# JohnsonLabJanelia/laserCalib

Hardware: NVIDIA B200
Metric: LM_iters_per_sec (higher is better)
Workload: dtype f64

## Files before the change

include/lcba.h:

```cpp
#ifndef LCBA_H
#define LCBA_H

#include <stddef.h>
#include <stdint.h>

#ifdef __cplusplus
extern "C" {
#endif

#define LCBA_VERSION 100
#define LCBA_CAM_PARAMS 11
#define LCBA_MAX_CAMERAS 64
#define LCBA_MAX_TRACE 512

enum {
  LCBA_OK = 0,
  LCBA_E_ARG = -1,
  LCBA_E_CUDA = -2,
  LCBA_E_STATE = -3,
  LCBA_E_UNSUPPORTED = -4,
  LCBA_E_NONFINITE = -5,
  LCBA_E_NCCL = -6
};

// ... 100 lines not shown

int lcba_nccl_unique_id(void* id_out128);
int lcba_comm_init(lcba_t* h, int32_t rank, int32_t nranks, const void* id128);

int lcba_debug_tr2d(double B00, double B01, double B11, double g0, double g1, double Delta,
                    double* p_out2, int* newton_out);

int lcba_debug_chol(lcba_t* h, int32_t n, const double* A, const double* rhs, double mu, const double* d,
                    int32_t grid, double* x_out, double* factor_out, int32_t* fail_out);

#define LCBA_STEP_SCALARS 18
int lcba_debug_step(lcba_t* h, double lam, double mu, int32_t mode, double* pc_out, double* pp_out,
                    double* scalars_out);

int lcba_debug_schur_stats(lcba_t* h, long long* out, int max_ctas, int* nkinds, int* nslices);

int lcba_debug_mma_plan(int32_t C, int32_t sm_count, int32_t* units_out, int32_t max_kinds,
                        int32_t* nslices_out, int32_t* ok_out);

int lcba_debug_i8_plan(int32_t C, int64_t P, int32_t sm_count, int32_t* tiles_out, int32_t max_tiles,
                       int32_t* work_out, int32_t max_work, int32_t* nwork_out, int32_t* nrg_out,
                       int64_t* nkb_out);

int lcba_debug_i8_fallback(lcba_t* h);

int lcba_debug_peer_reduce(lcba_t* h, int enable);

int lcba_host_is_nondecreasing_i64(const int64_t* v, int64_t n, int32_t threads);

#ifdef __cplusplus
}
#endif
#endif
```

lasercalib_b200/_cabi.py:

```python
from __future__ import annotations

import ctypes as C
import os

import numpy as np

_PKG = os.path.dirname(os.path.abspath(__file__))
LIB_PATH = os.path.join(_PKG, "liblcba.so")

LCBA_MAX_TRACE = 512
E_NAMES = {-1: "LCBA_E_ARG", -2: "LCBA_E_CUDA", -3: "LCBA_E_STATE", -4: "LCBA_E_UNSUPPORTED",
           -5: "LCBA_E_NONFINITE", -6: "LCBA_E_NCCL"}

SYMBOLS = ["lcba_version", "lcba_create", "lcba_destroy", "lcba_last_error", "lcba_default_options",
           "lcba_set_problem", "lcba_set_problem_shard", "lcba_set_params", "lcba_get_params", "lcba_rotate", "lcba_project",
           "lcba_unproject", "lcba_residuals", "lcba_jacobian_blocks", "lcba_sparsity_indices", "lcba_solve",
           "lcba_get_trace", "lcba_get_grad", "lcba_get_profile", "lcba_linearize",
           "lcba_time_device", "lcba_nccl_unique_id", "lcba_comm_init", "lcba_debug_tr2d",
           "lcba_sq_normal", "lcba_debug_schur_stats", "lcba_debug_mma_plan",
           "lcba_set_iteration_callback", "lcba_debug_i8_plan", "lcba_host_is_nondecreasing_i64", "lcba_debug_peer_reduce",
           "lcba_debug_i8_fallback", "lcba_debug_chol", "lcba_debug_step"]

STEP_SCALARS = ["reg_term", "Delta", "Jg2", "aa", "ab", "bb", "JAA", "JAB", "JBB", "gtgt", "gtp", "pp",
                "c0", "c1", "predicted", "step_h_norm", "step_norm", "chol_fail"]


class Options(C.Structure):
    _fields_ = [("ftol", C.c_double), ("xtol", C.c_double), ("gtol", C.c_double),
                ("max_nfev", C.c_int64), ("verbose", C.c_int32), ("profile", C.c_int32),
                ("max_iterations", C.c_int32), ("fix_cameras", C.c_int32), ("shared_intrinsics", C.c_int32), ("reserved", C.c_int32 * 3)]


class TraceRow(C.Structure):
    _fields_ = [("iteration", C.c_int64), ("nfev", C.c_int64), ("cost", C.c_double),
                ("cost_reduction", C.c_double), ("step_norm", C.c_double),
                ("optimality", C.c_double), ("delta", C.c_double), ("reg_term", C.c_double)]


class Result(C.Structure):
    _fields_ = [("cost", C.c_double), ("optimality", C.c_double), ("initial_cost", C.c_double),
                ("nfev", C.c_int64), ("njev", C.c_int64), ("iterations", C.c_int64),
                ("status", C.c_int32), ("n_trace", C.c_int32), ("solve_ms", C.c_double),
                ("gpu_launches", C.c_int64), ("reserved", C.c_double * 6)]

# ... 41 lines not shown
    lib.lcba_set_problem.argtypes = [vp, i32, i64, i64, vp, vp, vp, vp, vp, vp]
    lib.lcba_set_problem_shard.argtypes = [vp, i32, i64, i64, vp, vp, vp, vp, vp, vp, i64]
    lib.lcba_set_params.argtypes = [vp, vp, vp]
    lib.lcba_get_params.argtypes = [vp, vp, vp]
    lib.lcba_rotate.argtypes = [vp, i64, vp, vp, vp]
    lib.lcba_project.argtypes = [vp, i64, vp, vp, vp]
    lib.lcba_unproject.argtypes = [vp, i64, vp, vp, i64, vp, vp, vp, vp, vp]
    lib.lcba_residuals.argtypes = [vp, vp, vp, pd]
    lib.lcba_jacobian_blocks.argtypes = [vp, vp, vp, vp]
    lib.lcba_sparsity_indices.argtypes = [vp, i32, i64, i64, vp, vp, vp]
    lib.lcba_solve.argtypes = [vp, C.POINTER(Options), C.POINTER(Result)]
    lib.lcba_get_trace.argtypes = [vp, C.POINTER(TraceRow), i32]
    lib.lcba_set_iteration_callback.argtypes = [vp, ITERATION_CB, vp]
    lib.lcba_get_grad.argtypes = [vp, vp]
    lib.lcba_get_profile.argtypes = [vp, C.POINTER(KernelStat), i32, C.POINTER(i32)]
    lib.lcba_linearize.argtypes = [vp, dbl, vp, vp, vp, vp, pd]
    lib.lcba_time_device.argtypes = [vp, i32, i32, pd]
    lib.lcba_nccl_unique_id.argtypes = [vp]
    lib.lcba_comm_init.argtypes = [vp, i32, i32, vp]
    lib.lcba_sq_normal.argtypes = [vp, i32, vp, pd, vp, vp]
    lib.lcba_debug_mma_plan.argtypes = [i32, i32, vp, i32, C.POINTER(i32), C.POINTER(i32)]
    lib.lcba_debug_schur_stats.argtypes = [vp, vp, C.c_int, C.POINTER(C.c_int), C.POINTER(C.c_int)]
    lib.lcba_debug_i8_plan.argtypes = [i32, i64, i32, vp, i32, vp, i32, C.POINTER(i32), C.POINTER(i32), C.POINTER(i64)]
    lib.lcba_host_is_nondecreasing_i64.argtypes = [vp, i64, i32]
    lib.lcba_debug_peer_reduce.argtypes = [vp, i32]
    lib.lcba_debug_i8_fallback.argtypes = [vp]
    lib.lcba_debug_tr2d.argtypes = [dbl, dbl, dbl, dbl, dbl, dbl, pd, C.POINTER(C.c_int)]
    lib.lcba_debug_chol.argtypes = [vp, i32, vp, vp, dbl, vp, i32, vp, vp, C.POINTER(i32)]
    lib.lcba_debug_step.argtypes = [vp, dbl, dbl, i32, vp, vp, vp]
    _lib = lib
    return lib


def _ptr(a):
    return None if a is None else a.ctypes.data_as(C.c_void_p)


def _f64(a, shape=None):
    a = np.ascontiguousarray(a, dtype=np.float64)
    if shape is not None:
        a = a.reshape(shape)
    return a


def _i64(a):
    return np.ascontiguousarray(a, dtype=np.int64)
# ... 161 lines not shown
        return g

    def profile(self):
        stats = (KernelStat * 64)()
        n = C.c_int32()
        self._check(self.lib.lcba_get_profile(self.h, stats, 64, C.byref(n)))
        return {s.name.decode(): dict(launches=s.launches, total_ms=s.total_ms)
                for s in stats[:n.value]}

    def linearize(self, lam):
        n = 11 * self.C
        S = np.empty((n, n))
        rhs = np.empty(n)
        g = np.empty(n + 3 * self.P)
        sc = np.empty(n + 3 * self.P)
        cost = C.c_double()
        self._check(self.lib.lcba_linearize(self.h, float(lam), _ptr(S), _ptr(rhs), _ptr(g),
                                            _ptr(sc), C.byref(cost)))
        return dict(S=S, rhs=rhs, grad=g, scale_inv=sc, cost=cost.value)

    def i8_fell_back(self):
        return self.lib.lcba_debug_i8_fallback(self.h)

    def debug_chol(self, A, rhs, mu=0.0, d=None, grid=0):
        A = _f64(A)
        n = A.shape[0]
        if A.shape != (n, n):
            raise ValueError("A must be square")
        rhs = _f64(rhs).ravel()
        d = None if d is None else _f64(d).ravel()
        if rhs.size != n or (d is not None and d.size != n):
            raise ValueError("rhs and d must have n entries")
        x = np.empty(n)
        factor = np.empty((n + 1, n))
        fail = C.c_int32()
        self._check(self.lib.lcba_debug_chol(self.h, n, _ptr(A), _ptr(rhs), float(mu), _ptr(d), int(grid),
                                             _ptr(x), _ptr(factor), C.byref(fail)))
        return x, factor, fail.value

    STEP_FULL, STEP_FIX_CAMERAS, STEP_SHARED_INTRINSICS = 0, 1, 2

    def debug_step(self, lam, mu=0.0, mode=0):
        pc = np.empty(11 * self.C)
        pp = np.empty(3 * self.P)
        sc = np.empty(len(STEP_SCALARS))
        self._check(self.lib.lcba_debug_step(self.h, float(lam), float(mu), int(mode), _ptr(pc), _ptr(pp), _ptr(sc)))
# ... 28 lines not shown
```

lasercalib_b200/csrc/lcba.cu:

```cuda
#include <dlfcn.h>
#include <math.h>
#include <stdio.h>
#include <string.h>
#include <algorithm>
#include <map>
#include <string>
#include <thread>
#include <vector>

#include <nvtx3/nvToolsExt.h>

#include "common.cuh"
#include "control.cuh"
#include "dense.cuh"
#include "eval.cuh"
#include "ingest.cuh"
#include "linearize.cuh"
#include "dense_passes.cuh"
#include "schur.cuh"
#include "schur_mma.cuh"
#include "schur_i8.cuh"
#include "peer_reduce.cuh"
#include "variants.cuh"

// ... 504 lines not shown
  h->plan = make_schur_plan(C, h->sm_count, h->smem_optin - 2048);
  LCBA_TRY(dev_alloc(h, &h->d_kinds, h->plan.kinds.size()));
  LCBA_TRY(dev_alloc(h, &h->d_hws, h->plan.hws.size()));
  LCBA_CUDA(h, cudaMemcpyAsync(h->d_kinds, h->plan.kinds.data(), h->plan.kinds.size() * sizeof(SchurKind),
                               cudaMemcpyHostToDevice, st));
  LCBA_CUDA(h, cudaMemcpyAsync(h->d_hws, h->plan.hws.data(), h->plan.hws.size() * sizeof(SchurHw),
                               cudaMemcpyHostToDevice, st));
  LCBA_TRY(dev_alloc(h, &h->d_Sred, h->plan.part_stride));
  h->use_mma = false;
  h->d_mkinds = nullptr; h->d_U = nullptr; h->d_Upart = nullptr; h->d_Yg = nullptr;
  int max_slices = h->plan.nslices;
  {
    const char* de = getenv("LCBA_MMA_DENSITY");
    const double min_density = de ? atof(de) : 0.25;
    const bool dense = (double)h->n_pairs >= min_density * (double)P * C;
    const char* env = getenv("LCBA_SCHUR_MMA");
    const bool want = env ? atoi(env) != 0 : (dense && C >= 8);
    if (want && C <= MMA_MAX_CAMERAS) {
      {
        const char* ie = getenv("LCBA_SCHUR_I8");
        h->use_i8 = ie ? atoi(ie) != 0 : P >= 32768;
      }
      if (h->use_i8) {
        h->i8plan = make_i8_plan(C, P, h->sm_count);
        const I8Plan& ip = h->i8plan;
        h->i8_groups = (C + I8_GROUP_CAMS - 1) / I8_GROUP_CAMS;
        h->i8_gx_max = (int)std::max<long long>(1, std::min<long long>(ip.nkb, (long long)h->sm_count * 4 / h->i8_groups));
        h->i8_gx_make = (int)std::max<long long>(1, std::min<long long>(ip.nkb, (long long)h->sm_count * 3 / h->i8_groups));
        LCBA_TRY(dev_alloc(h, &h->d_i8work, ip.work.size()));
        LCBA_TRY(dev_alloc(h, &h->d_i8tiles, ip.tiles.size()));
        LCBA_CUDA(h, cudaMemcpyAsync(h->d_i8work, ip.work.data(), ip.work.size() * sizeof(I8Work), cudaMemcpyHostToDevice, st));
        LCBA_CUDA(h, cudaMemcpyAsync(h->d_i8tiles, ip.tiles.data(), ip.tiles.size() * sizeof(I8Tile), cudaMemcpyHostToDevice, st));
        LCBA_TRY(dev_alloc(h, &h->d_i8planes, ip.plane_bytes));
        {
          const char* te = getenv("LCBA_I8_TMA");
          h->i8_tma = !(te && atoi(te) == 0) && i8_encode_maps(ip, h->d_i8planes, &h->i8maps);
          if (!h->i8_tma) memset(&h->i8maps, 0, sizeof(h->i8maps));
        }
        LCBA_TRY(dev_alloc(h, &h->d_i8partial, ip.work.size() * 128 * 64));
        LCBA_TRY(dev_alloc(h, &h->d_i8rmax, (size_t)h->i8_gx_max * ip.NRG * 8));
        LCBA_TRY(dev_alloc(h, &h->d_i8erow, (size_t)ip.NRG * 8));
        LCBA_TRY(dev_alloc(h, &h->d_i8gate, 1));
        LCBA_TRY(dev_alloc(h, &h->d_i8mrow, (size_t)ip.NRG * 8));
        LCBA_CUDA(h, cudaMemsetAsync(h->d_i8gate, 0, sizeof(int), st));
        {
          const char* ge = getenv("LCBA_I8_GUARD");
          h->i8_guard = !(ge && atoi(ge) == 0);
// ... 333 lines not shown
          h->d_tab[w], h->d_pts[w], h->d_pair_w, h->d_pair_start, h->d_mask, h->P, C, h->camn_pb, h->d_Upart));
    KL(h, "reduce", k_reduce_cols<<<nblk(C * CAMN_VALS, RC_COLS), RC_COLS * RC_ROWS, 0, h->stream>>>(
          h->d_Upart, h->camn_grid, C * CAMN_VALS, h->d_U));
    }
    const int nt = (NCP * C + 1 + 7) / 8, last = nt - 6 * ((nt + 5) / 6 - 1);
    if (h->use_i8) {
      const I8Plan& ip = h->i8plan;
      const int RP = ip.NRG * 8;
      const size_t smem_rm = ((size_t)I8_GROUP_CAMS * CAMTAB + 192) * 4;
      KL(h, "i8_rowmax", k_i8_rowmax<<<dim3(h->i8_gx_max, h->i8_groups), 192, smem_rm, h->stream>>>(
            h->d_tab[w], h->d_pts[w], h->d_pair_w, h->d_pair_start, h->d_mask, h->d_Lz, h->P, C, RP, h->d_i8rmax));
      KL(h, "i8_rowmax", k_i8_rowexp<<<nblk(RP, 128), 128, 0, h->stream>>>(h->d_i8rmax, h->i8_gx_max, NCP * C + 1, RP,
                                                                     h->d_i8erow, h->d_i8mrow));
      KL(h, "make_Y", k_i8_make<<<dim3(h->i8_gx_make, h->i8_groups), 192, i8_make_smem_bytes(), h->stream>>>(
            h->d_tab[w], h->d_pts[w], h->d_pair_w, h->d_pair_start, h->d_mask, h->d_Lz, h->P, C, ip.NRG, h->d_i8erow,
            h->d_i8planes));
      if (h->i8_tma)
        KL(h, "schur", k_i8_syrk<true><<<(unsigned)ip.work.size(), I8_THREADS, ip.smem_bytes, h->stream>>>(
              h->i8maps, h->d_i8planes, ip.NRG, h->d_i8work, h->d_i8partial, h->d_fail, h->d_stats));
      else
        KL(h, "schur", k_i8_syrk<false><<<(unsigned)ip.work.size(), I8_THREADS, ip.smem_bytes, h->stream>>>(
              h->i8maps, h->d_i8planes, ip.NRG, h->d_i8work, h->d_i8partial, h->d_fail, h->d_stats));
      KL(h, "schur_reduce", k_i8_gather<<<dim3((unsigned)ip.tiles.size(), 16), 256, 0, h->stream>>>(
            h->d_i8partial, h->d_i8tiles, C, h->d_i8erow, pl.npairs, h->d_Sred));
      KL(h, "schur_reduce", k_add_cam_blocks<<<nblk(C * 121, 128), 128, 0, h->stream>>>(h->d_U, C, h->d_Sred));
      if (h->i8_guard) {
        KL(h, "i8_check", k_i8_check<<<1, 256, 0, h->stream>>>(h->d_i8mrow, C, h->d_Sred, h->d_i8gate));
#define LCBA_MMA_GATED(L)                                                                            \
  KL(h, "i8_fallback", (k_schur_mma<L, false><<<dim3(mp.nslices, mp.nkinds), MMA_THREADS, mp.smem_bytes, h->stream>>>( \
          nullptr, h->d_tab[w], h->d_pts[w], h->d_pair_w, h->d_pair_start, h->d_mask, h->d_Lz, h->P, h->n_pairs, C, \
          h->d_mkinds, mp.nslices, pl.part_stride, pl.npairs, h->d_Spart, nullptr, h->d_i8gate)))
        switch (last) {
          case 1: LCBA_MMA_GATED(1); break;
          case 2: LCBA_MMA_GATED(2); break;
          case 3: LCBA_MMA_GATED(3); break;
          case 4: LCBA_MMA_GATED(4); break;
          case 5: LCBA_MMA_GATED(5); break;
          default: LCBA_MMA_GATED(6); break;
        }
#undef LCBA_MMA_GATED
        KL(h, "i8_fallback", k_i8_fallback_finish<<<h->sm_count, 256, 0, h->stream>>>(
              h->d_i8gate, h->d_Spart, mp.nslices, pl.part_stride, h->d_U, C, h->d_Sred));
      }
    } else {
    if (h->d_Yg) {
      const int pbk = MAKEY_THREADS / C, rpk = mp.kinds[0].rp;
      const size_t smem_y = ((size_t)((C * CAMTAB + 1) & ~1) + (size_t)3 * pbk * rpk) * 8;
// ... 643 lines not shown
  return pl.nkinds;
}

extern "C" int lcba_debug_i8_plan(int32_t C, int64_t P, int32_t sm_count, int32_t* tiles_out, int32_t max_tiles,
                                  int32_t* work_out, int32_t max_work, int32_t* nwork_out, int32_t* nrg_out,
                                  int64_t* nkb_out) {
  if (C < 1 || C > LCBA_MAX_CAMERAS || P < 1 || !tiles_out) return LCBA_E_ARG;
  const I8Plan pl = make_i8_plan(C, P, sm_count);
  for (size_t i = 0; i < pl.tiles.size() && (int)i < max_tiles; ++i) {
    const I8Tile& t = pl.tiles[i];
    int32_t* o = tiles_out + 8 * i;
    o[0] = t.m_rg0; o[1] = t.m_nrg; o[2] = t.n_rg0; o[3] = t.n_nrg; o[4] = t.n2_rg0; o[5] = t.n2_nrg; o[6] = t.w0; o[7] = t.nw;
  }
  if (work_out)
    for (size_t i = 0; i < pl.work.size() && (int)i < max_work; ++i) {
      work_out[3 * i] = (int32_t)i; work_out[3 * i + 1] = pl.work[i].kb0; work_out[3 * i + 2] = pl.work[i].kb1;
    }
  if (nwork_out) *nwork_out = (int32_t)pl.work.size();
  if (nrg_out) *nrg_out = pl.NRG;
  if (nkb_out) *nkb_out = pl.nkb;
  return (int)pl.tiles.size();
}

extern "C" int lcba_sq_normal(lcba_t* h, int32_t mode, const double* theta, double* cost_out,
                              double* g_out, double* H_out) {
  if (!h || !h->have_problem) { set_error(h, "lcba_sq_normal: no problem set"); return LCBA_E_STATE; }
  if (!theta || (mode != LCBA_SQ_CAMONLY && mode != LCBA_SQ_TRANSFORM) || ((g_out == nullptr) != (H_out == nullptr))) {
    set_error(h, "lcba_sq_normal: bad mode, NULL theta, or only one of g / H given");
    return LCBA_E_ARG;
  }
  cudaSetDevice(h->device);
  const int C = h->C;
  const bool derivs = g_out != nullptr;
  const int K = (mode == LCBA_SQ_CAMONLY ? C * SQC_VALS : SQT_VALS) + 1;
  const int warps = sq_camonly_warps(C, h->smem_optin);
  const int threads = (mode == LCBA_SQ_CAMONLY) ? warps * 32 : SQ_THREADS;
  const int per_sm = (mode == LCBA_SQ_CAMONLY) ? 1 : 2;
  const int grid = (int)std::max<long long>(1, std::min<long long>((h->N + threads - 1) / threads,
                                                                   (long long)h->sm_count * per_sm));
  if (!h->d_sqpart || h->sq_grid < grid || h->sq_K < K) {
    LCBA_TRY(dev_alloc(h, &h->d_sqpart, (size_t)grid * K));
    LCBA_TRY(dev_alloc(h, &h->d_sqout, (size_t)K));
    if (!h->d_theta) LCBA_TRY(dev_alloc(h, &h->d_theta, 16));
    h->sq_grid = grid;
    h->sq_K = K;
  }
// ... 171 lines not shown
```

lasercalib_b200/csrc/schur_i8.cuh:

```cuda
#pragma once
#include <cuda.h>
#include <algorithm>
#include <vector>
#include "common.cuh"
#include "schur_mma.cuh"

namespace lcba {

constexpr int I8_NS = 6;
constexpr int I8_DMAX = 6;
constexpr int I8_ND = I8_DMAX + 1;
constexpr int I8_PTS = 21;
constexpr int I8_STAGES = 3;
constexpr int I8_FLUSH = 224;
constexpr int I8_THREADS = 192;
constexpr int I8_RG_BYTES = 512;
constexpr int I8_GROUP_CAMS = 8;
constexpr int I8_GROUP_RG = 13;
constexpr int I8_GROUP_ROWS = I8_GROUP_RG * 8;

struct I8Work {
  int m_rg0, m_nrg, n_rg0, n_nrg, n2_rg0, n2_nrg;
  int kb0, kb1;
  int map_a, map_b1, map_b2, pad;
};
constexpr int I8_MAX_MAPS = 6;
struct alignas(64) I8Maps { CUtensorMap m[I8_MAX_MAPS]; };
struct I8Tile { int m_rg0, m_nrg, n_rg0, n_nrg, n2_rg0, n2_nrg, w0, nw; };

struct I8Plan {
  int C = 0, R = 0, NRG = 0;
  long long nkb = 0;
  int map_heights[I8_MAX_MAPS] = {0, 0, 0, 0, 0, 0};
  int nmaps = 0;
  std::vector<I8Tile> tiles;
  std::vector<I8Work> work;
  size_t plane_bytes = 0, smem_bytes = 0;
};

inline I8Plan make_i8_plan(int C, long long P, int sm_count) {
  I8Plan pl;
  pl.C = C;
  pl.R = NCP * C + 1;
  pl.NRG = (pl.R + 7) / 8;
  pl.NRG += pl.NRG & 1;
  pl.nkb = (P + I8_PTS - 1) / I8_PTS;
  const int NRG = pl.NRG;
  const int nmt = (NRG + 15) / 16;
  const int last_m = NRG - 16 * (nmt - 1);
  const bool fold = nmt > 1 && last_m <= 4;
  const int nfull = fold ? nmt - 1 : nmt;
  const int col_w = fold ? 8 - last_m : 8;
  const int c0 = 16 * (nmt - 1);
  for (int mt = 0; mt < nfull; ++mt) {
    const int m0 = 16 * mt, mn = std::min(16, NRG - m0);
    for (int n0 = 0; n0 < m0 + mn; n0 += col_w) {
      const int nn = std::min(col_w, m0 + mn - n0);
      const bool last = n0 + col_w >= m0 + mn;
      I8Tile t{m0, mn, n0, nn, fold && last ? c0 : 0, fold && last ? last_m : 0, 0, 0};
      pl.tiles.push_back(t);
    }
  }
  if (fold) {
    I8Tile t{c0, last_m, c0, last_m, 0, 0, 0, 0};
    pl.tiles.push_back(t);
  }
  auto block_cost = [](int nrg) { return nrg <= 0 ? 0.0 : (nrg <= 2 ? 592.0 : (nrg <= 4 ? 812.0 : (nrg <= 6 ? 1181.0 : 1550.0))); };
  std::vector<double> cost(pl.tiles.size());
  std::vector<long long> nr(pl.tiles.size(), 1);
  for (size_t ti = 0; ti < pl.tiles.size(); ++ti) cost[ti] = 507.0 + block_cost(pl.tiles[ti].n_nrg) + block_cost(pl.tiles[ti].n2_nrg);
  for (long long left = (long long)sm_count - (long long)pl.tiles.size(); left > 0; --left) {
    size_t worst = 0;
    double tw = -1.0;
    for (size_t ti = 0; ti < pl.tiles.size(); ++ti) {
      const double tt = nr[ti] < pl.nkb ? cost[ti] / (double)nr[ti] : -1.0;
      if (tt > tw) { tw = tt; worst = ti; }
    }
    if (tw < 0.0) break;
    ++nr[worst];
  }
  for (size_t ti = 0; ti < pl.tiles.size(); ++ti) {
    I8Tile& t = pl.tiles[ti];
    const long long n = std::min<long long>(nr[ti], pl.nkb);
    t.w0 = (int)pl.work.size();
    t.nw = (int)n;
    auto map_of = [&](int h) {
      if (h == 0) return 0;
      for (int i = 0; i < pl.nmaps && i < I8_MAX_MAPS; ++i) if (pl.map_heights[i] == h) return i;
      if (pl.nmaps < I8_MAX_MAPS) pl.map_heights[pl.nmaps] = h;
      return pl.nmaps++;
    };
    const int ma = map_of(t.m_nrg), mb1 = map_of(t.n_nrg), mb2 = map_of(t.n2_nrg);
    for (long long q = 0; q < n; ++q) {
      I8Work w{t.m_rg0, t.m_nrg, t.n_rg0, t.n_nrg, t.n2_rg0, t.n2_nrg, (int)(pl.nkb * q / n), (int)(pl.nkb * (q + 1) / n),
               ma, mb1, mb2, 0};
      pl.work.push_back(w);
    }
  }
  pl.plane_bytes = (size_t)pl.nkb * I8_NS * NRG * I8_RG_BYTES;
  pl.smem_bytes = (size_t)I8_STAGES * I8_NS * (16 + 8) * I8_RG_BYTES + 1024;
  return pl;
}

inline bool i8_encode_maps(const I8Plan& pl, void* planes, I8Maps* out) {
  if (pl.nmaps <= 0 || pl.nmaps > I8_MAX_MAPS) return false;
  typedef CUresult (*EncodeFn)(CUtensorMap*, CUtensorMapDataType, cuuint32_t, void*, const cuuint64_t*, const cuuint64_t*,
                               const cuuint32_t*, const cuuint32_t*, CUtensorMapInterleave, CUtensorMapSwizzle,
                               CUtensorMapL2promotion, CUtensorMapFloatOOBfill);
  void* fn = nullptr;
  cudaDriverEntryPointQueryResult qres;
  if (cudaGetDriverEntryPoint("cuTensorMapEncodeTiled", &fn, cudaEnableDefault, &qres) != cudaSuccess || !fn ||
      qres != cudaDriverEntryPointSuccess) {
    cudaGetLastError();
    return false;
  }
  const cuuint64_t gdim[4] = {128, (cuuint64_t)pl.NRG, (cuuint64_t)I8_NS, (cuuint64_t)pl.nkb};
  const cuuint64_t gstr[3] = {(cuuint64_t)I8_RG_BYTES, (cuuint64_t)pl.NRG * I8_RG_BYTES, (cuuint64_t)I8_NS * pl.NRG * I8_RG_BYTES};
  const cuuint32_t estr[4] = {1, 1, 1, 1};
  memset(out, 0, sizeof(*out));
  for (int i = 0; i < pl.nmaps; ++i) {
    const cuuint32_t box[4] = {128, (cuuint32_t)pl.map_heights[i], (cuuint32_t)I8_NS, 1};
    const CUresult r = ((EncodeFn)fn)(&out->m[i], CU_TENSOR_MAP_DATA_TYPE_UINT32, 4, planes, gdim, gstr, box, estr,
                                      CU_TENSOR_MAP_INTERLEAVE_NONE, CU_TENSOR_MAP_SWIZZLE_NONE,
                                      CU_TENSOR_MAP_L2_PROMOTION_L2_256B, CU_TENSOR_MAP_FLOAT_OOB_FILL_NONE);
    if (r != CUDA_SUCCESS) return false;
  }
  return true;
}

__device__ __forceinline__ void i8_tma_4d(uint32_t dst, const CUtensorMap* map, int c0, int c1, int c2, int c3, uint32_t bar) {
  asm volatile("cp.async.bulk.tensor.4d.shared::cluster.global.mbarrier::complete_tx::bytes [%0], [%1, {%2, %3, %4, %5}], [%6];"
               ::"r"(dst), "l"(map), "r"(c0), "r"(c1), "r"(c2), "r"(c3), "r"(bar) : "memory");
}
__device__ __forceinline__ uint32_t i8_smem_u32(const void* p) { return (uint32_t)__cvta_generic_to_shared(p); }
__device__ __forceinline__ void i8_mbar_init(uint32_t bar, uint32_t count) {
  asm volatile("mbarrier.init.shared::cta.b64 [%0], %1;" ::"r"(bar), "r"(count) : "memory");
}
__device__ __forceinline__ void i8_mbar_expect_tx(uint32_t bar, uint32_t bytes) {
  asm volatile("mbarrier.arrive.expect_tx.shared::cta.b64 _, [%0], %1;" ::"r"(bar), "r"(bytes) : "memory");
}
__device__ __forceinline__ void i8_mbar_arrive(uint32_t bar) {
  asm volatile("mbarrier.arrive.shared::cta.b64 _, [%0];" ::"r"(bar) : "memory");
}
template <bool BACKOFF>
__device__ __forceinline__ void i8_mbar_wait(uint32_t bar, uint32_t parity, int* fail) {
  const long long t0 = clock64();
  while (true) {
    uint32_t ok;
    asm volatile("{\n\t.reg .pred p;\n\tmbarrier.try_wait.parity.shared::cta.b64 p, [%1], %2;\n\tselp.u32 %0, 1, 0, p;\n\t}"
                 : "=r"(ok) : "r"(bar), "r"(parity) : "memory");
    if (ok) return;
    if (BACKOFF) __nanosleep(128);
    if (clock64() - t0 > 6000000000LL) { atomicOr(fail, 4); asm volatile("trap;"); }
  }
}
// ... 352 lines not shown
#pragma unroll
  for (int ks = 0; ks < 2; ++ks) {
    const uint32_t o = 256u * ks;
    if (ks == 0 && first) {
      i8_issue_kstep<NCOL1, true>(tmem, sA + o, sB1 + o, a_bytes, b1_bytes);
      if (NCOL2 > 0) i8_issue_kstep<NCOL2 ? NCOL2 : 16, true>(tmem + I8_ND * NCOL1, sA + o, sB2 + o, a_bytes, b2_bytes);
    } else {
      i8_issue_kstep<NCOL1, false>(tmem, sA + o, sB1 + o, a_bytes, b1_bytes);
      if (NCOL2 > 0) i8_issue_kstep<NCOL2 ? NCOL2 : 16, false>(tmem + I8_ND * NCOL1, sA + o, sB2 + o, a_bytes, b2_bytes);
    }
  }
}

template <bool TMA>
__global__ void __launch_bounds__(I8_THREADS, 1)
k_i8_syrk(const __grid_constant__ I8Maps maps, const unsigned char* __restrict__ planes, int NRG,
          const I8Work* __restrict__ work, double* __restrict__ partial, int* __restrict__ fail,
          long long* __restrict__ stats ) {
  extern __shared__ __align__(1024) uint8_t i8_smem[];
  __shared__ __align__(8) uint64_t s_bar[2 * I8_STAGES + 2];
  __shared__ uint32_t s_tmem;
  const I8Work W = work[blockIdx.x];
  const int tid = threadIdx.x, wid = tid >> 5, lane = tid & 31;
  const uint32_t a_bytes = (uint32_t)W.m_nrg * I8_RG_BYTES, b_bytes = (uint32_t)W.n_nrg * I8_RG_BYTES;
  const uint32_t b2_bytes = (uint32_t)W.n2_nrg * I8_RG_BYTES;
  const uint32_t B2_OFF = (uint32_t)I8_NS * b_bytes;
  constexpr uint32_t A_REGION = (uint32_t)I8_NS * 16 * I8_RG_BYTES;
  constexpr uint32_t STAGE_BYTES = (uint32_t)I8_NS * (16 + 8) * I8_RG_BYTES;
  const uint32_t smem0 = i8_smem_u32(i8_smem);
  const uint32_t bar_full = i8_smem_u32(&s_bar[0]), bar_empty = i8_smem_u32(&s_bar[I8_STAGES]);
  const uint32_t bar_tfull = i8_smem_u32(&s_bar[2 * I8_STAGES]), bar_tempty = i8_smem_u32(&s_bar[2 * I8_STAGES + 1]);
  const int ncol = W.n_nrg * 8, ncol2 = W.n2_nrg * 8;
  if (tid == 0) {
    for (int s = 0; s < I8_STAGES; ++s) { i8_mbar_init(bar_full + 8 * s, 1); i8_mbar_init(bar_empty + 8 * s, 1); }
    i8_mbar_init(bar_tfull, 1);
    i8_mbar_init(bar_tempty, 128);
    asm volatile("fence.mbarrier_init.release.cluster;" ::: "memory");
  }
  if (wid == 5) {
    asm volatile("tcgen05.alloc.cta_group::1.sync.aligned.shared::cta.b32 [%0], %1;" ::"r"(i8_smem_u32(&s_tmem)), "r"(512u) : "memory");
    asm volatile("tcgen05.relinquish_alloc_permit.cta_group::1.sync.aligned;" ::: "memory");
  }
  asm volatile("tcgen05.fence::before_thread_sync;" ::: "memory");
  __syncthreads();
  asm volatile("tcgen05.fence::after_thread_sync;" ::: "memory");
  const uint32_t tmem = s_tmem;
  const int nkb = W.kb1 - W.kb0;

  if (wid == 4) {
    if (TMA) {
      if (lane == 0) {
        for (int it = 0; it < nkb; ++it) {
          const int st = it % I8_STAGES;
          if (it >= I8_STAGES) i8_mbar_wait<false>(bar_empty + 8 * st, ((it / I8_STAGES) - 1) & 1, fail);
          i8_mbar_expect_tx(bar_full + 8 * st, (uint32_t)I8_NS * (a_bytes + b_bytes + b2_bytes));
          const uint32_t dstA = smem0 + st * STAGE_BYTES, dstB = dstA + A_REGION;
          const int kb = W.kb0 + it;
          i8_tma_4d(dstA, &maps.m[W.map_a], 0, W.m_rg0, 0, kb, bar_full + 8 * st);
          i8_tma_4d(dstB, &maps.m[W.map_b1], 0, W.n_rg0, 0, kb, bar_full + 8 * st);
          if (W.n2_nrg > 0) i8_tma_4d(dstB + B2_OFF, &maps.m[W.map_b2], 0, W.n2_rg0, 0, kb, bar_full + 8 * st);
        }
      }
    } else {
    const int ci = lane / 3, cb = lane - 3 * ci;
    const bool mine = lane < 3 * I8_NS && (cb < 2 || W.n2_nrg > 0);
    for (int it = 0; it < nkb; ++it) {
      const int st = it % I8_STAGES;
      if (it >= I8_STAGES) i8_mbar_wait<false>(bar_empty + 8 * st, ((it / I8_STAGES) - 1) & 1, fail);
      if (lane == 0) i8_mbar_expect_tx(bar_full + 8 * st, (uint32_t)I8_NS * (a_bytes + b_bytes + b2_bytes));
      __syncwarp();
      if (mine) {
        const unsigned char* src = planes + (size_t)(W.kb0 + it) * I8_NS * NRG * I8_RG_BYTES + (size_t)ci * NRG * I8_RG_BYTES;
        const uint32_t dstA = smem0 + st * STAGE_BYTES, dstB = dstA + A_REGION;
        if (cb == 0) i8_bulk_g2s(dstA + ci * a_bytes, src + (size_t)W.m_rg0 * I8_RG_BYTES, a_bytes, bar_full + 8 * st);
        else if (cb == 1) i8_bulk_g2s(dstB + ci * b_bytes, src + (size_t)W.n_rg0 * I8_RG_BYTES, b_bytes, bar_full + 8 * st);
        else i8_bulk_g2s(dstB + B2_OFF + ci * b2_bytes, src + (size_t)W.n2_rg0 * I8_RG_BYTES, b2_bytes, bar_full + 8 * st);
      }
    }
    }
  } else if (wid == 5) {
    if (i8_elect_one()) {
      int since_flush = 0, nflush = 0;
      long long t_wait = 0;
      const long long t_begin = stats ? clock64() : 0;
      for (int it = 0; it < nkb; ++it) {
        const int st = it % I8_STAGES;
        if (since_flush == 0 && nflush > 0) {
          i8_mbar_wait<false>(bar_tempty, (nflush - 1) & 1, fail);
          asm volatile("tcgen05.fence::after_thread_sync;" ::: "memory");
        }
        if (stats) {
          const long long w0 = clock64();
          i8_mbar_wait<false>(bar_full + 8 * st, (it / I8_STAGES) & 1, fail);
          t_wait += clock64() - w0;
        } else {
          i8_mbar_wait<false>(bar_full + 8 * st, (it / I8_STAGES) & 1, fail);
        }
        asm volatile("tcgen05.fence::after_thread_sync;" ::: "memory");
// ... 47 lines not shown
            for (int c = 0; c < 16; ++c) acc[16 * h + c] = fma((double)(int)v[c], sc, acc[16 * h + c]);
          } else if (16 * h >= 64 - ncol2) {
            uint32_t v[16];
            i8_tmem_ld16(tmem + ((uint32_t)(q * 32) << 16) + (uint32_t)(I8_ND * ncol + d * ncol2 + 16 * h - (64 - ncol2)), v);
            asm volatile("tcgen05.wait::ld.sync.aligned;" ::: "memory");
#pragma unroll
            for (int c = 0; c < 16; ++c) acc[16 * h + c] = fma((double)(int)v[c], sc, acc[16 * h + c]);
          }
        }
      }
      asm volatile("tcgen05.fence::before_thread_sync;" ::: "memory");
      i8_mbar_arrive(bar_tempty);
    }
    double* out = partial + ((size_t)blockIdx.x * 128 + row) * 64;
#pragma unroll
    for (int c = 0; c < 64; ++c) out[c] = acc[c];
  }
  asm volatile("tcgen05.fence::before_thread_sync;" ::: "memory");
  __syncthreads();
  if (wid == 5) asm volatile("tcgen05.dealloc.cta_group::1.sync.aligned.b32 %0, %1;" ::"r"(tmem), "r"(512u) : "memory");
}

__global__ void __launch_bounds__(256)
k_i8_gather(const double* __restrict__ partial, const I8Tile* __restrict__ tiles, int C,
            const int* __restrict__ e_row, int npairs, double* __restrict__ Sred) {
  const I8Tile T = tiles[blockIdx.x];
  const int n = NCP * C;
  const int nr = T.m_nrg * 8, nc1 = T.n_nrg * 8, nc2 = T.n2_nrg * 8, nc = nc1 + nc2;
  for (int idx = threadIdx.x + blockDim.x * blockIdx.y; idx < nr * nc; idx += blockDim.x * gridDim.y) {
    const int tr = idx / nc, tcl = idx - tr * nc;
    const bool second = tcl >= nc1;
    const int tc = second ? 64 - nc2 + (tcl - nc1) : tcl;
    int rho = T.m_rg0 * 8 + tr, sig = second ? T.n2_rg0 * 8 + (tcl - nc1) : T.n_rg0 * 8 + tcl;
    if (second) { const int x = rho; rho = sig; sig = x; }
    if (rho > n || sig >= n || sig > rho) continue;
    double s = 0.0;
    for (int w = 0; w < T.nw; ++w) s += partial[((size_t)(T.w0 + w) * 128 + tr) * 64 + tc];
    const double v = -ldexp(s, e_row[rho] + e_row[sig]);
    const int ck = sig / NCP, cb = sig % NCP;
    if (rho == n) { Sred[(size_t)npairs * 121 + ck * NCP + cb] = v; continue; }
    const int cj = rho / NCP, ra = rho % NCP;
    double* blk = Sred + (size_t)(cj * (cj + 1) / 2 + ck) * 121;
    blk[ra * NCP + cb] = v;
    if (cj == ck && ra != cb) blk[cb * NCP + ra] = v;
  }
}

constexpr double I8_RHO_MAX = 16.0;
__global__ void __launch_bounds__(256)
k_i8_check(const double* __restrict__ m_row, int C, const double* __restrict__ Sred, int* __restrict__ gate) {
  int bad = 0;
  for (int r = threadIdx.x; r < NCP * C; r += blockDim.x) {
    const double m = m_row[r];
    if (m > 0.0) {
      const int c = r / NCP, a = r % NCP;
      const double d = Sred[(size_t)(c * (c + 1) / 2 + c) * 121 + a * NCP + a];
      if (!(m * m <= I8_RHO_MAX * d)) bad = 1;
    }
// ... 29 lines not shown
```

Before: 129.6.

## Add cover-based int8 Schur tile plan with two-segment A tiles, chosen by cost model

Adds an alternative tiling for the int8 tcgen05 Schur SYRK. It pairs 8-row-group blocks so each tile loads two non-adjacent A row segments, using a 5D TMA map with a stride delta or an extra bulk copy lane, to cover the lower triangle with fewer redundant columns. A cycle cost model picks between the existing strip plan and the cover plan, and an env var can force either one. The gather kernel now handles the two-segment rows and deduplicates mirrored entries. This adds complexity in TMA map encoding and in index logic that could be wrong.

```diff
diff --git a/include/lcba.h b/include/lcba.h
--- a/include/lcba.h
+++ b/include/lcba.h
@@ -146,6 +146,10 @@
                        int32_t* work_out, int32_t max_work, int32_t* nwork_out, int32_t* nrg_out,
                        int64_t* nkb_out);
 
+int lcba_debug_i8_cover_plan(int32_t C, int64_t P, int32_t sm_count, int32_t which, int32_t* tiles_out,
+                             int32_t max_tiles, int32_t* work_out, int32_t max_work, int32_t* nwork_out,
+                             int32_t* nrg_out, int64_t* nkb_out, int32_t* cover_out, double* model_out);
+
 int lcba_debug_i8_fallback(lcba_t* h);
 
 int lcba_debug_peer_reduce(lcba_t* h, int enable);
diff --git a/lasercalib_b200/_cabi.py b/lasercalib_b200/_cabi.py
--- a/lasercalib_b200/_cabi.py
+++ b/lasercalib_b200/_cabi.py
@@ -19,7 +19,7 @@
            "lcba_time_device", "lcba_nccl_unique_id", "lcba_comm_init", "lcba_debug_tr2d",
            "lcba_sq_normal", "lcba_debug_schur_stats", "lcba_debug_mma_plan",
            "lcba_set_iteration_callback", "lcba_debug_i8_plan", "lcba_host_is_nondecreasing_i64", "lcba_debug_peer_reduce",
-           "lcba_debug_i8_fallback", "lcba_debug_chol", "lcba_debug_step"]
+           "lcba_debug_i8_fallback", "lcba_debug_chol", "lcba_debug_step", "lcba_debug_i8_cover_plan"]
 
 STEP_SCALARS = ["reg_term", "Delta", "Jg2", "aa", "ab", "bb", "JAA", "JAB", "JBB", "gtgt", "gtp", "pp",
                 "c0", "c1", "predicted", "step_h_norm", "step_norm", "chol_fail"]
@@ -107,6 +107,8 @@
     lib.lcba_debug_mma_plan.argtypes = [i32, i32, vp, i32, C.POINTER(i32), C.POINTER(i32)]
     lib.lcba_debug_schur_stats.argtypes = [vp, vp, C.c_int, C.POINTER(C.c_int), C.POINTER(C.c_int)]
     lib.lcba_debug_i8_plan.argtypes = [i32, i64, i32, vp, i32, vp, i32, C.POINTER(i32), C.POINTER(i32), C.POINTER(i64)]
+    lib.lcba_debug_i8_cover_plan.argtypes = [i32, i64, i32, i32, vp, i32, vp, i32, C.POINTER(i32), C.POINTER(i32),
+                                             C.POINTER(i64), C.POINTER(i32), vp]
     lib.lcba_host_is_nondecreasing_i64.argtypes = [vp, i64, i32]
     lib.lcba_debug_peer_reduce.argtypes = [vp, i32]
     lib.lcba_debug_i8_fallback.argtypes = [vp]
@@ -314,6 +316,24 @@
     def i8_fell_back(self):
         return self.lib.lcba_debug_i8_fallback(self.h)
 
+    I8_PLAN_CHOSEN, I8_PLAN_STRIP, I8_PLAN_COVER = 0, 1, 2
+
+    @staticmethod
+    def i8_plan(n_cams, P, sm_count, which=0):
+        lib = load()
+        tiles = np.zeros((512, 10), dtype=np.int32)
+        work = np.zeros((1024, 3), dtype=np.int32)
+        nwork, nrg, nkb, cover = C.c_int32(), C.c_int32(), C.c_int64(), C.c_int32()
+        model = np.zeros(4)
+        nt = lib.lcba_debug_i8_cover_plan(int(n_cams), int(P), int(sm_count), int(which), _ptr(tiles), tiles.shape[0],
+                                          _ptr(work), work.shape[0], C.byref(nwork), C.byref(nrg), C.byref(nkb),
+                                          C.byref(cover), _ptr(model))
+        if nt < 0:
+            raise LcbaError(nt, "lcba_debug_i8_cover_plan: bad arguments")
+        return dict(tiles=tiles[:nt].copy(), work=work[:nwork.value].copy(), nrg=nrg.value, nkb=nkb.value,
+                    cover=bool(cover.value), executed_ops=model[0], cycles=model[1], strip_cycles=model[2],
+                    cover_cycles=model[3])
+
     def debug_chol(self, A, rhs, mu=0.0, d=None, grid=0):
         A = _f64(A)
         n = A.shape[0]
diff --git a/lasercalib_b200/csrc/lcba.cu b/lasercalib_b200/csrc/lcba.cu
--- a/lasercalib_b200/csrc/lcba.cu
+++ b/lasercalib_b200/csrc/lcba.cu
@@ -550,7 +550,11 @@
         h->use_i8 = ie ? atoi(ie) != 0 : P >= 32768;
       }
       if (h->use_i8) {
-        h->i8plan = make_i8_plan(C, P, h->sm_count);
+        {
+          const char* pe = getenv("LCBA_I8_PLAN");
+          const int which = !pe ? 0 : (strcmp(pe, "strip") == 0 ? 1 : (strcmp(pe, "cover") == 0 ? 2 : 0));
+          h->i8plan = make_i8_best_plan(C, P, h->sm_count, which);
+        }
         const I8Plan& ip = h->i8plan;
         h->i8_groups = (C + I8_GROUP_CAMS - 1) / I8_GROUP_CAMS;
         h->i8_gx_max = (int)std::max<long long>(1, std::min<long long>(ip.nkb, (long long)h->sm_count * 4 / h->i8_groups));
@@ -930,7 +934,7 @@
         KL(h, "schur", k_i8_syrk<false><<<(unsigned)ip.work.size(), I8_THREADS, ip.smem_bytes, h->stream>>>(
               h->i8maps, h->d_i8planes, ip.NRG, h->d_i8work, h->d_i8partial, h->d_fail, h->d_stats));
       KL(h, "schur_reduce", k_i8_gather<<<dim3((unsigned)ip.tiles.size(), 16), 256, 0, h->stream>>>(
-            h->d_i8partial, h->d_i8tiles, C, h->d_i8erow, pl.npairs, h->d_Sred));
+            h->d_i8partial, h->d_i8tiles, C, ip.cover ? 1 : 0, h->d_i8erow, pl.npairs, h->d_Sred));
       KL(h, "schur_reduce", k_add_cam_blocks<<<nblk(C * 121, 128), 128, 0, h->stream>>>(h->d_U, C, h->d_Sred));
       if (h->i8_guard) {
         KL(h, "i8_check", k_i8_check<<<1, 256, 0, h->stream>>>(h->d_i8mrow, C, h->d_Sred, h->d_i8gate));
@@ -1620,6 +1624,37 @@
   return (int)pl.tiles.size();
 }
 
+extern "C" int lcba_debug_i8_cover_plan(int32_t C, int64_t P, int32_t sm_count, int32_t which, int32_t* tiles_out,
+                                        int32_t max_tiles, int32_t* work_out, int32_t max_work, int32_t* nwork_out,
+                                        int32_t* nrg_out, int64_t* nkb_out, int32_t* cover_out, double* model_out) {
+  if (C < 1 || C > LCBA_MAX_CAMERAS || P < 1 || sm_count < 1 || which < 0 || which > 2 || !tiles_out) return LCBA_E_ARG;
+  const I8Plan pl = make_i8_best_plan(C, P, sm_count, which);
+  for (size_t i = 0; i < pl.tiles.size() && (int)i < max_tiles; ++i) {
+    const I8Tile& t = pl.tiles[i];
+    int32_t* o = tiles_out + 10 * i;
+    o[0] = t.m_rg0; o[1] = t.m_nrg; o[2] = t.m2_rg0; o[3] = t.m2_nrg; o[4] = t.n_rg0; o[5] = t.n_nrg;
+    o[6] = t.n2_rg0; o[7] = t.n2_nrg; o[8] = t.w0; o[9] = t.nw;
+  }
+  if (work_out)
+    for (size_t i = 0; i < pl.work.size() && (int)i < max_work; ++i) {
+      const I8Work& w = pl.work[i];
+      int ti = 0;
+      while (ti + 1 < (int)pl.tiles.size() && pl.tiles[ti + 1].w0 <= (int)i) ++ti;
+      work_out[3 * i] = ti; work_out[3 * i + 1] = w.kb0; work_out[3 * i + 2] = w.kb1;
+    }
+  if (nwork_out) *nwork_out = (int32_t)pl.work.size();
+  if (nrg_out) *nrg_out = pl.NRG;
+  if (nkb_out) *nkb_out = pl.nkb;
+  if (cover_out) *cover_out = pl.cover ? 1 : 0;
+  if (model_out) {
+    model_out[0] = i8_executed_ops(pl);
+    model_out[1] = pl.model_cycles;
+    model_out[2] = make_i8_plan(C, P, sm_count).model_cycles;
+    model_out[3] = make_i8_cover_plan(C, P, sm_count).model_cycles;
+  }
+  return (int)pl.tiles.size();
+}
+
 extern "C" int lcba_sq_normal(lcba_t* h, int32_t mode, const double* theta, double* cost_out,
                               double* g_out, double* H_out) {
   if (!h || !h->have_problem) { set_error(h, "lcba_sq_normal: no problem set"); return LCBA_E_STATE; }
diff --git a/lasercalib_b200/csrc/schur_i8.cuh b/lasercalib_b200/csrc/schur_i8.cuh
--- a/lasercalib_b200/csrc/schur_i8.cuh
+++ b/lasercalib_b200/csrc/schur_i8.cuh
@@ -20,31 +20,83 @@
 constexpr int I8_GROUP_ROWS = I8_GROUP_RG * 8;
 
 struct I8Work {
-  int m_rg0, m_nrg, n_rg0, n_nrg, n2_rg0, n2_nrg;
+  int m_rg0, m_nrg, m2_rg0, m2_nrg, n_rg0, n_nrg, n2_rg0, n2_nrg;
   int kb0, kb1;
   int map_a, map_b1, map_b2, pad;
 };
-constexpr int I8_MAX_MAPS = 6;
+constexpr int I8_MAX_MAPS = 16;
 struct alignas(64) I8Maps { CUtensorMap m[I8_MAX_MAPS]; };
-struct I8Tile { int m_rg0, m_nrg, n_rg0, n_nrg, n2_rg0, n2_nrg, w0, nw; };
+struct I8Tile { int m_rg0, m_nrg, m2_rg0, m2_nrg, n_rg0, n_nrg, n2_rg0, n2_nrg, w0, nw; };
 
 struct I8Plan {
   int C = 0, R = 0, NRG = 0;
   long long nkb = 0;
-  int map_heights[I8_MAX_MAPS] = {0, 0, 0, 0, 0, 0};
+  int map_heights[I8_MAX_MAPS] = {};
+  int map_delta[I8_MAX_MAPS] = {};
   int nmaps = 0;
+  bool cover = false;
+  double model_cycles = 0.0;
   std::vector<I8Tile> tiles;
   std::vector<I8Work> work;
   size_t plane_bytes = 0, smem_bytes = 0;
 };
 
-inline I8Plan make_i8_plan(int C, long long P, int sm_count) {
+inline double i8_block_cost(int nrg) {
+  return nrg <= 0 ? 0.0 : (nrg <= 2 ? 592.0 : (nrg <= 4 ? 812.0 : (nrg <= 6 ? 1181.0 : 1550.0)));
+}
+inline double i8_tile_cost(const I8Tile& t) { return 507.0 + i8_block_cost(t.n_nrg) + i8_block_cost(t.n2_nrg); }
+
+inline void i8_deal(I8Plan& pl, int sm_count) {
+  std::vector<double> cost(pl.tiles.size());
+  std::vector<long long> nr(pl.tiles.size(), 1);
+  for (size_t ti = 0; ti < pl.tiles.size(); ++ti) cost[ti] = i8_tile_cost(pl.tiles[ti]);
+  for (long long left = (long long)sm_count - (long long)pl.tiles.size(); left > 0; --left) {
+    size_t worst = 0;
+    double tw = -1.0;
+    for (size_t ti = 0; ti < pl.tiles.size(); ++ti) {
+      const double tt = nr[ti] < pl.nkb ? cost[ti] / (double)nr[ti] : -1.0;
+      if (tt > tw) { tw = tt; worst = ti; }
+    }
+    if (tw < 0.0) break;
+    ++nr[worst];
+  }
+  pl.model_cycles = 0.0;
+  for (size_t ti = 0; ti < pl.tiles.size(); ++ti) {
+    I8Tile& t = pl.tiles[ti];
+    const long long n = std::min<long long>(nr[ti], pl.nkb);
+    t.w0 = (int)pl.work.size();
+    t.nw = (int)n;
+    auto map_of = [&](int h, int delta) {
+      if (h == 0) return 0;
+      for (int i = 0; i < pl.nmaps && i < I8_MAX_MAPS; ++i)
+        if (pl.map_heights[i] == h && pl.map_delta[i] == delta) return i;
+      if (pl.nmaps < I8_MAX_MAPS) { pl.map_heights[pl.nmaps] = h; pl.map_delta[pl.nmaps] = delta; }
+      return pl.nmaps++;
+    };
+    const int ma = map_of(t.m_nrg, t.m2_nrg > 0 ? t.m2_rg0 - t.m_rg0 : 0), mb1 = map_of(t.n_nrg, 0), mb2 = map_of(t.n2_nrg, 0);
+    for (long long q = 0; q < n; ++q) {
+      I8Work w{t.m_rg0, t.m_nrg, t.m2_rg0, t.m2_nrg, t.n_rg0, t.n_nrg, t.n2_rg0, t.n2_nrg,
+               (int)(pl.nkb * q / n), (int)(pl.nkb * (q + 1) / n), ma, mb1, mb2, 0};
+      pl.work.push_back(w);
+    }
+    pl.model_cycles = std::max(pl.model_cycles, cost[ti] * (double)((pl.nkb + n - 1) / n));
+  }
+  pl.plane_bytes = (size_t)pl.nkb * I8_NS * pl.NRG * I8_RG_BYTES;
+  pl.smem_bytes = (size_t)I8_STAGES * I8_NS * (16 + 8) * I8_RG_BYTES + 1024;
+}
+
+inline I8Plan i8_plan_base(int C, long long P) {
   I8Plan pl;
   pl.C = C;
   pl.R = NCP * C + 1;
   pl.NRG = (pl.R + 7) / 8;
   pl.NRG += pl.NRG & 1;
   pl.nkb = (P + I8_PTS - 1) / I8_PTS;
+  return pl;
+}
+
+inline I8Plan make_i8_plan(int C, long long P, int sm_count) {
+  I8Plan pl = i8_plan_base(C, P);
   const int NRG = pl.NRG;
   const int nmt = (NRG + 15) / 16;
   const int last_m = NRG - 16 * (nmt - 1);
@@ -57,49 +109,66 @@
     for (int n0 = 0; n0 < m0 + mn; n0 += col_w) {
       const int nn = std::min(col_w, m0 + mn - n0);
       const bool last = n0 + col_w >= m0 + mn;
-      I8Tile t{m0, mn, n0, nn, fold && last ? c0 : 0, fold && last ? last_m : 0, 0, 0};
+      I8Tile t{m0, mn, 0, 0, n0, nn, fold && last ? c0 : 0, fold && last ? last_m : 0, 0, 0};
       pl.tiles.push_back(t);
     }
   }
   if (fold) {
-    I8Tile t{c0, last_m, c0, last_m, 0, 0, 0, 0};
+    I8Tile t{c0, last_m, 0, 0, c0, last_m, 0, 0, 0, 0};
     pl.tiles.push_back(t);
   }
-  auto block_cost = [](int nrg) { return nrg <= 0 ? 0.0 : (nrg <= 2 ? 592.0 : (nrg <= 4 ? 812.0 : (nrg <= 6 ? 1181.0 : 1550.0))); };
-  std::vector<double> cost(pl.tiles.size());
-  std::vector<long long> nr(pl.tiles.size(), 1);
-  for (size_t ti = 0; ti < pl.tiles.size(); ++ti) cost[ti] = 507.0 + block_cost(pl.tiles[ti].n_nrg) + block_cost(pl.tiles[ti].n2_nrg);
-  for (long long left = (long long)sm_count - (long long)pl.tiles.size(); left > 0; --left) {
-    size_t worst = 0;
-    double tw = -1.0;
-    for (size_t ti = 0; ti < pl.tiles.size(); ++ti) {
-      const double tt = nr[ti] < pl.nkb ? cost[ti] / (double)nr[ti] : -1.0;
-      if (tt > tw) { tw = tt; worst = ti; }
-    }
-    if (tw < 0.0) break;
-    ++nr[worst];
-  }
-  for (size_t ti = 0; ti < pl.tiles.size(); ++ti) {
-    I8Tile& t = pl.tiles[ti];
-    const long long n = std::min<long long>(nr[ti], pl.nkb);
-    t.w0 = (int)pl.work.size();
-    t.nw = (int)n;
-    auto map_of = [&](int h) {
-      if (h == 0) return 0;
-      for (int i = 0; i < pl.nmaps && i < I8_MAX_MAPS; ++i) if (pl.map_heights[i] == h) return i;
-      if (pl.nmaps < I8_MAX_MAPS) pl.map_heights[pl.nmaps] = h;
-      return pl.nmaps++;
-    };
-    const int ma = map_of(t.m_nrg), mb1 = map_of(t.n_nrg), mb2 = map_of(t.n2_nrg);
-    for (long long q = 0; q < n; ++q) {
-      I8Work w{t.m_rg0, t.m_nrg, t.n_rg0, t.n_nrg, t.n2_rg0, t.n2_nrg, (int)(pl.nkb * q / n), (int)(pl.nkb * (q + 1) / n),
-               ma, mb1, mb2, 0};
-      pl.work.push_back(w);
-    }
-  }
-  pl.plane_bytes = (size_t)pl.nkb * I8_NS * NRG * I8_RG_BYTES;
-  pl.smem_bytes = (size_t)I8_STAGES * I8_NS * (16 + 8) * I8_RG_BYTES + 1024;
+  i8_deal(pl, sm_count);
   return pl;
+}
+
+inline I8Plan make_i8_cover_plan(int C, long long P, int sm_count) {
+  I8Plan pl = i8_plan_base(C, P);
+  pl.cover = true;
+  const int G = pl.NRG / 8, r = pl.NRG - 8 * G;
+  std::vector<std::vector<int>> to(G);
+  for (int b = 0; b < G; ++b)
+    for (int a = 0; a < b; ++a) to[b].push_back(a);
+  std::vector<int> even;
+  for (int z = 0; z < G; ++z) if (to[z].size() % 2 == 0) even.push_back(z);
+  for (size_t k = 0; k + 1 < even.size(); k += 2) {
+    const int u = even[k], v = even[k + 1];
+    to[v].erase(std::find(to[v].begin(), to[v].end(), u));
+    to[u].push_back(v);
+  }
+  auto tile = [&](int x, int y, int j0, int jn) {
+    int a = std::min(x, y < 0 ? x : y), b = std::max(x, y);
+    I8Tile t{8 * a, 8, 0, 0, j0, jn, 0, 0, 0, 0};
+    if (y >= 0 && b == a + 1) t.m_nrg = 16;
+    else if (y >= 0) { t.m2_rg0 = 8 * b; t.m2_nrg = 8; }
+    pl.tiles.push_back(t);
+  };
+  for (int z = 0; z < G; ++z) {
+    std::vector<int> items(1, z);
+    items.insert(items.end(), to[z].begin(), to[z].end());
+    std::sort(items.begin() + 1, items.end());
+    for (size_t k = 0; k < items.size(); k += 2) tile(items[k], k + 1 < items.size() ? items[k + 1] : -1, 8 * z, 8);
+  }
+  if (r > 0) {
+    if (G > 0) pl.tiles.push_back(I8Tile{8 * (G - 1), 8 + r, 0, 0, 8 * G, r, 0, 0, 0, 0});
+    else pl.tiles.push_back(I8Tile{0, r, 0, 0, 0, r, 0, 0, 0, 0});
+    for (int x = 0; x + 1 < G; x += 2) tile(x, x + 2 < G ? x + 1 : -1, 8 * G, r);
+  }
+  i8_deal(pl, sm_count);
+  return pl;
+}
+
+inline I8Plan make_i8_best_plan(int C, long long P, int sm_count, int which) {
+  if (which == 1) return make_i8_plan(C, P, sm_count);
+  I8Plan cv = make_i8_cover_plan(C, P, sm_count);
+  if (which == 2) return cv;
+  I8Plan st = make_i8_plan(C, P, sm_count);
+  return cv.model_cycles < st.model_cycles ? cv : st;
+}
+
+inline double i8_executed_ops(const I8Plan& pl) {
+  long long cols = 0;
+  for (const I8Tile& t : pl.tiles) cols += 8 * (t.n_nrg + t.n2_nrg);
+  return 26.0 * 2.0 * 128.0 * (double)cols * 64.0 * (double)pl.nkb;
 }
 
 inline bool i8_encode_maps(const I8Plan& pl, void* planes, I8Maps* out) {
@@ -114,15 +183,27 @@
     cudaGetLastError();
     return false;
   }
-  const cuuint64_t gdim[4] = {128, (cuuint64_t)pl.NRG, (cuuint64_t)I8_NS, (cuuint64_t)pl.nkb};
-  const cuuint64_t gstr[3] = {(cuuint64_t)I8_RG_BYTES, (cuuint64_t)pl.NRG * I8_RG_BYTES, (cuuint64_t)I8_NS * pl.NRG * I8_RG_BYTES};
-  const cuuint32_t estr[4] = {1, 1, 1, 1};
+  const cuuint64_t rg = I8_RG_BYTES, slice = (cuuint64_t)pl.NRG * I8_RG_BYTES, blk = (cuuint64_t)I8_NS * slice;
+  const cuuint32_t estr[5] = {1, 1, 1, 1, 1};
   memset(out, 0, sizeof(*out));
   for (int i = 0; i < pl.nmaps; ++i) {
-    const cuuint32_t box[4] = {128, (cuuint32_t)pl.map_heights[i], (cuuint32_t)I8_NS, 1};
-    const CUresult r = ((EncodeFn)fn)(&out->m[i], CU_TENSOR_MAP_DATA_TYPE_UINT32, 4, planes, gdim, gstr, box, estr,
-                                      CU_TENSOR_MAP_INTERLEAVE_NONE, CU_TENSOR_MAP_SWIZZLE_NONE,
-                                      CU_TENSOR_MAP_L2_PROMOTION_L2_256B, CU_TENSOR_MAP_FLOAT_OOB_FILL_NONE);
+    const cuuint32_t h = (cuuint32_t)pl.map_heights[i];
+    CUresult r;
+    if (pl.map_delta[i] == 0) {
+      const cuuint64_t gdim[4] = {128, (cuuint64_t)pl.NRG, (cuuint64_t)I8_NS, (cuuint64_t)pl.nkb};
+      const cuuint64_t gstr[3] = {rg, slice, blk};
+      const cuuint32_t box[4] = {128, h, (cuuint32_t)I8_NS, 1};
+      r = ((EncodeFn)fn)(&out->m[i], CU_TENSOR_MAP_DATA_TYPE_UINT32, 4, planes, gdim, gstr, box, estr,
+                         CU_TENSOR_MAP_INTERLEAVE_NONE, CU_TENSOR_MAP_SWIZZLE_NONE,
+                         CU_TENSOR_MAP_L2_PROMOTION_L2_256B, CU_TENSOR_MAP_FLOAT_OOB_FILL_NONE);
+    } else {
+      const cuuint64_t gdim[5] = {128, (cuuint64_t)(pl.NRG - pl.map_delta[i]), 2, (cuuint64_t)I8_NS, (cuuint64_t)pl.nkb};
+      const cuuint64_t gstr[4] = {rg, (cuuint64_t)pl.map_delta[i] * rg, slice, blk};
+      const cuuint32_t box[5] = {128, h, 2, (cuuint32_t)I8_NS, 1};
+      r = ((EncodeFn)fn)(&out->m[i], CU_TENSOR_MAP_DATA_TYPE_UINT32, 5, planes, gdim, gstr, box, estr,
+                         CU_TENSOR_MAP_INTERLEAVE_NONE, CU_TENSOR_MAP_SWIZZLE_NONE,
+                         CU_TENSOR_MAP_L2_PROMOTION_L2_256B, CU_TENSOR_MAP_FLOAT_OOB_FILL_NONE);
+    }
     if (r != CUDA_SUCCESS) return false;
   }
   return true;
@@ -131,6 +212,10 @@
 __device__ __forceinline__ void i8_tma_4d(uint32_t dst, const CUtensorMap* map, int c0, int c1, int c2, int c3, uint32_t bar) {
   asm volatile("cp.async.bulk.tensor.4d.shared::cluster.global.mbarrier::complete_tx::bytes [%0], [%1, {%2, %3, %4, %5}], [%6];"
                ::"r"(dst), "l"(map), "r"(c0), "r"(c1), "r"(c2), "r"(c3), "r"(bar) : "memory");
+}
+__device__ __forceinline__ void i8_tma_5d(uint32_t dst, const CUtensorMap* map, int c0, int c1, int c2, int c3, int c4, uint32_t bar) {
+  asm volatile("cp.async.bulk.tensor.5d.shared::cluster.global.mbarrier::complete_tx::bytes [%0], [%1, {%2, %3, %4, %5, %6}], [%7];"
+               ::"r"(dst), "l"(map), "r"(c0), "r"(c1), "r"(c2), "r"(c3), "r"(c4), "r"(bar) : "memory");
 }
 __device__ __forceinline__ uint32_t i8_smem_u32(const void* p) { return (uint32_t)__cvta_generic_to_shared(p); }
 __device__ __forceinline__ void i8_mbar_init(uint32_t bar, uint32_t count) {
@@ -529,7 +614,8 @@
   __shared__ uint32_t s_tmem;
   const I8Work W = work[blockIdx.x];
   const int tid = threadIdx.x, wid = tid >> 5, lane = tid & 31;
-  const uint32_t a_bytes = (uint32_t)W.m_nrg * I8_RG_BYTES, b_bytes = (uint32_t)W.n_nrg * I8_RG_BYTES;
+  const uint32_t a1_bytes = (uint32_t)W.m_nrg * I8_RG_BYTES, a_bytes = a1_bytes + (uint32_t)W.m2_nrg * I8_RG_BYTES;
+  const uint32_t b_bytes = (uint32_t)W.n_nrg * I8_RG_BYTES;
   const uint32_t b2_bytes = (uint32_t)W.n2_nrg * I8_RG_BYTES;
   const uint32_t B2_OFF = (uint32_t)I8_NS * b_bytes;
   constexpr uint32_t A_REGION = (uint32_t)I8_NS * 16 * I8_RG_BYTES;
@@ -563,14 +649,15 @@
           i8_mbar_expect_tx(bar_full + 8 * st, (uint32_t)I8_NS * (a_bytes + b_bytes + b2_bytes));
           const uint32_t dstA = smem0 + st * STAGE_BYTES, dstB = dstA + A_REGION;
           const int kb = W.kb0 + it;
-          i8_tma_4d(dstA, &maps.m[W.map_a], 0, W.m_rg0, 0, kb, bar_full + 8 * st);
+          if (W.m2_nrg > 0) i8_tma_5d(dstA, &maps.m[W.map_a], 0, W.m_rg0, 0, 0, kb, bar_full + 8 * st);
+          else i8_tma_4d(dstA, &maps.m[W.map_a], 0, W.m_rg0, 0, kb, bar_full + 8 * st);
           i8_tma_4d(dstB, &maps.m[W.map_b1], 0, W.n_rg0, 0, kb, bar_full + 8 * st);
           if (W.n2_nrg > 0) i8_tma_4d(dstB + B2_OFF, &maps.m[W.map_b2], 0, W.n2_rg0, 0, kb, bar_full + 8 * st);
         }
       }
     } else {
-    const int ci = lane / 3, cb = lane - 3 * ci;
-    const bool mine = lane < 3 * I8_NS && (cb < 2 || W.n2_nrg > 0);
+    const int ci = lane / 4, cb = lane - 4 * ci;
+    const bool mine = lane < 4 * I8_NS && (cb == 0 || cb == 2 || (cb == 1 && W.m2_nrg > 0) || (cb == 3 && W.n2_nrg > 0));
     for (int it = 0; it < nkb; ++it) {
       const int st = it % I8_STAGES;
       if (it >= I8_STAGES) i8_mbar_wait<false>(bar_empty + 8 * st, ((it / I8_STAGES) - 1) & 1, fail);
@@ -579,8 +666,9 @@
       if (mine) {
         const unsigned char* src = planes + (size_t)(W.kb0 + it) * I8_NS * NRG * I8_RG_BYTES + (size_t)ci * NRG * I8_RG_BYTES;
         const uint32_t dstA = smem0 + st * STAGE_BYTES, dstB = dstA + A_REGION;
-        if (cb == 0) i8_bulk_g2s(dstA + ci * a_bytes, src + (size_t)W.m_rg0 * I8_RG_BYTES, a_bytes, bar_full + 8 * st);
-        else if (cb == 1) i8_bulk_g2s(dstB + ci * b_bytes, src + (size_t)W.n_rg0 * I8_RG_BYTES, b_bytes, bar_full + 8 * st);
+        if (cb == 0) i8_bulk_g2s(dstA + ci * a_bytes, src + (size_t)W.m_rg0 * I8_RG_BYTES, a1_bytes, bar_full + 8 * st);
+        else if (cb == 1) i8_bulk_g2s(dstA + ci * a_bytes + a1_bytes, src + (size_t)W.m2_rg0 * I8_RG_BYTES, a_bytes - a1_bytes, bar_full + 8 * st);
+        else if (cb == 2) i8_bulk_g2s(dstB + ci * b_bytes, src + (size_t)W.n_rg0 * I8_RG_BYTES, b_bytes, bar_full + 8 * st);
         else i8_bulk_g2s(dstB + B2_OFF + ci * b2_bytes, src + (size_t)W.n2_rg0 * I8_RG_BYTES, b2_bytes, bar_full + 8 * st);
       }
     }
@@ -674,18 +762,24 @@
 }
 
 __global__ void __launch_bounds__(256)
-k_i8_gather(const double* __restrict__ partial, const I8Tile* __restrict__ tiles, int C,
+k_i8_gather(const double* __restrict__ partial, const I8Tile* __restrict__ tiles, int C, int cover,
             const int* __restrict__ e_row, int npairs, double* __restrict__ Sred) {
   const I8Tile T = tiles[blockIdx.x];
   const int n = NCP * C;
-  const int nr = T.m_nrg * 8, nc1 = T.n_nrg * 8, nc2 = T.n2_nrg * 8, nc = nc1 + nc2;
+  const int nr1 = T.m_nrg * 8, nr = nr1 + T.m2_nrg * 8, nc1 = T.n_nrg * 8, nc2 = T.n2_nrg * 8, nc = nc1 + nc2;
   for (int idx = threadIdx.x + blockDim.x * blockIdx.y; idx < nr * nc; idx += blockDim.x * gridDim.y) {
     const int tr = idx / nc, tcl = idx - tr * nc;
     const bool second = tcl >= nc1;
     const int tc = second ? 64 - nc2 + (tcl - nc1) : tcl;
-    int rho = T.m_rg0 * 8 + tr, sig = second ? T.n2_rg0 * 8 + (tcl - nc1) : T.n_rg0 * 8 + tcl;
-    if (second) { const int x = rho; rho = sig; sig = x; }
-    if (rho > n || sig >= n || sig > rho) continue;
+    int rho = tr < nr1 ? T.m_rg0 * 8 + tr : T.m2_rg0 * 8 + (tr - nr1);
+    int sig = second ? T.n2_rg0 * 8 + (tcl - nc1) : T.n_rg0 * 8 + tcl;
+    if (rho < sig) {
+      const int g = sig >> 3, gr = rho >> 3;
+      const bool col_in_rows = (g >= T.m_rg0 && g < T.m_rg0 + T.m_nrg) || (g >= T.m2_rg0 && g < T.m2_rg0 + T.m2_nrg);
+      if (col_in_rows && (!cover || (gr >= T.n_rg0 && gr < T.n_rg0 + T.n_nrg))) continue;
+      const int x = rho; rho = sig; sig = x;
+    }
+    if (rho > n || sig >= n) continue;
     double s = 0.0;
     for (int w = 0; w < T.nw; ++w) s += partial[((size_t)(T.w0 + w) * 128 + tr) * 64 + tc];
     const double v = -ldexp(s, e_row[rho] + e_row[sig]);
```

Measured after the change: 137.3 (median of 6 runs). 6.0% higher.
